# hpcaitech/CachedEmbedding

Hardware: AMD Instinct MI355X
Metric: embedding lookups/sec (cache op + EmbeddingBag fwd + bwd/SGD), Criteo-1TB table @1% cache (higher is better)
Workload: dtype f32

## Files before the change

cachedembedding_amd/_lib.py:

```python
from __future__ import annotations

import ctypes
import os
from ctypes import POINTER, Structure, c_char_p, c_double, c_float, c_int, c_int32, c_int64, c_size_t, c_uint64, c_void_p
from pathlib import Path

import torch

_PKG = Path(__file__).resolve().parent
LIB_PATH = Path(os.environ["CE_LIBRARY"]) if os.environ.get("CE_LIBRARY") else _PKG / "libce_hip.so"

CE_OK = 0
CE_ERR_INVALID = 1
CE_ERR_HIP = 2
CE_ERR_CAPACITY = 3
CE_ERR_NOMEM = 4
CE_ERR_UNSUPPORTED = 5
CE_ERR_RANGE = 6
CE_EVICT_DATASET = 0
CE_EVICT_LFU = 1
CE_EVICT_LRU = 2
CE_MODE_SUM = 0
CE_MODE_MEAN = 1
CE_ACT_F32 = 0
CE_ACT_BF16 = 1
CE_ACT_F16 = 2
CE_OPT_SGD = 0
CE_OPT_ROWWISE_ADAGRAD = 1
CE_ROUND_NEAREST = 0
CE_ROUND_STOCHASTIC = 1
CE_SORTED_CHUNK = 64
CE_COMPACT_BLOCK = 4096
CE_ACC_CACHE = 0
CE_ACC_STEP = 1
CE_WD_NONE = 0
CE_WD_L2 = 1
CE_WD_DECOUPLED = 2
CE_TRANSPORT_ZEROCOPY = 0
CE_TRANSPORT_STAGED = 1
CE_TRANSPORT_WORKER = 2
CE_CALL_PREPARE = 0
CE_CALL_PRELOAD = 1
CE_CALL_FLUSH = 2
CE_Q8_HEADER_BYTES = 16
CE_Q4_HEADER_BYTES = 16


class CeCacheConfig(Structure):
    _fields_ = [
        ("num_embeddings", c_int64),
        ("cuda_row_num", c_int64),
        ("embedding_dim", c_int32),
        ("evict_strategy", c_int32),
        ("transport", c_int32),
        ("protect_depth", c_int32),
        ("max_ids_per_call", c_int64),
        ("host_weight", c_void_p),
        ("host_weight_dev", c_void_p),
        ("cache_weight", c_void_p),
        ("idx_map", c_void_p),
        ("inverted_cached_idx", c_void_p),
        ("cached_idx_map", c_void_p),
        ("freq_cnter", c_void_p),
        ("workspace", c_void_p),
        ("workspace_bytes", c_size_t),
    ]


class CeCallStats(Structure):
    _fields_ = [
# ... 25 lines not shown
_WD = [c_float, c_int32]
_UPDATE_WD_TAIL = _KEYS + [c_void_p, c_void_p, c_int64, c_float, c_void_p, c_float] + _WD + \
    [c_int32, c_int32, c_uint64, c_int32, c_void_p, c_size_t] + _STREAM
_SORTED_WD_TAIL = [c_void_p, c_void_p, c_int64, c_float, c_float] + _WD + \
    [c_int32, c_int32, c_uint64, c_void_p, c_size_t] + _STREAM
_ADAM_WD_TAIL = _KEYS + [c_double, c_double, c_float, c_void_p, c_float] + _WD + \
    [c_void_p, c_int32, c_void_p, c_size_t] + _STREAM
_ROW_MOMENT = [c_void_p, c_void_p, c_int64]
_WINDOW = [c_void_p, c_int64, c_int64, c_int64]
_WINDOW_SRC = _WINDOW + [c_void_p, c_int32, c_int64, c_int64, c_int32, c_int64]
SIGNATURES = {
    "ce_version": (c_int, []),
    "ce_cpu_budget": (c_int32, []),
    "ce_last_error": (c_char_p, []),
    "ce_stream_create_cu_mask": (c_int, [c_void_p, c_int32, POINTER(c_void_p)]),
    "ce_stream_destroy": (c_int, [c_void_p]),
    "ce_host_alloc": (c_int, [c_size_t, c_int, POINTER(c_void_p), POINTER(c_void_p)]),
    "ce_host_free": (c_int, [c_void_p]),
    "ce_host_register": (c_int, [c_void_p, c_size_t, POINTER(c_void_p)]),
    "ce_host_unregister": (c_int, [c_void_p]),
    "ce_host_fill_uniform": (c_int, [c_void_p, c_int64, c_float, c_float, c_uint64, c_int]),
    "ce_host_fill_uniform_rows": (c_int, [c_void_p, c_int64, c_int32, c_float, c_float, c_uint64, c_void_p, c_void_p]),
    "ce_host_rows_gather": (c_int, [c_void_p, c_int64, c_int32, c_void_p, c_int64, c_void_p, c_void_p]),
    "ce_box_probe": (c_int, [c_void_p, c_size_t, c_int32, POINTER(c_double), POINTER(c_double), c_void_p]),
    "ce_probe_rows": (c_int, [c_void_p, c_int64, c_int32, c_int64, c_int32, POINTER(c_double), POINTER(c_double), c_void_p]),
    "ce_bag_forward": (c_int, _BAG + _STREAM),
    "ce_bag_backward_dense": (c_int, _BAG + _STREAM),
    "ce_bag_backward_dense_presorted": (c_int, _BAG + _KEYS + _STREAM),
    "ce_bag_backward_rows": (c_int, [c_void_p, c_void_p, c_int32, c_int64, c_void_p, c_int32, c_int64, c_int32, c_void_p,
                                     c_int32, c_int64, c_void_p, c_void_p]),
    "ce_bag_backward_sgd": (c_int, _BAG + [c_float] + _STREAM),
    "ce_bag_presort_len": (c_int64, [c_int64]),
    "ce_bag_presort": (c_int, [c_void_p, c_int64, c_int64, c_void_p, c_void_p]),
    "ce_bag_backward_sgd_presorted": (c_int, _BAG + [c_float] + _KEYS + _STREAM),
    "ce_bag_presort_window": (c_int, _WINDOW + _KEYS + _STREAM),
    "ce_bag_presort_window_src": (c_int, _WINDOW_SRC + _KEYS + _STREAM),
    "ce_bag_forward_src_keys": (c_int, _TABLE + [c_int64] + _KEYS + [c_void_p] + _STREAM),
    "ce_bag_backward_sgd_presorted_src": (c_int, _SRC + [c_float] + _KEYS + _STREAM),
    "ce_bag_presort_window_src_excl": (c_int, _WINDOW_SRC + [c_void_p] + _KEYS + [c_void_p] + _STREAM),
    "ce_bag_backward_sgd_presorted_src_excl": (c_int, _SRC + [c_float] + _KEYS + [c_void_p] + _STREAM),
    "ce_bag_backward_dense_presorted_src": (c_int, _SRC + _KEYS + _STREAM),
    "ce_bag_backward_sgd_sorted_workspace": (c_size_t, [c_int64, c_int64]),
    "ce_bag_backward_sgd_sorted": (c_int, _BAG + [c_float, c_void_p, c_size_t] + _STREAM),
    "ce_bag_backward_rowwise_adagrad_workspace": (c_size_t, [c_int64, c_int32]),
    "ce_bag_backward_rowwise_adagrad": (c_int, _BAG + _ADAGRAD_TAIL),
    "ce_bag_backward_rowwise_adagrad_src": (c_int, _SRC + _ADAGRAD_TAIL),
    "ce_bag_forward_act": (c_int, _BAG + _ACT + _STREAM),
    "ce_bag_forward_src_keys_act": (c_int, _TABLE + [c_int64] + _KEYS + [c_void_p] + _ACT + _STREAM),
    "ce_bag_backward_dense_act": (c_int, _BAG + _ACT + _KEYS + _STREAM),
    "ce_bag_backward_sgd_act": (c_int, _BAG + _ACT + [c_float] + _KEYS + _STREAM),
    "ce_bag_backward_sgd_src_act": (c_int, _SRC + _ACT + [c_float] + _KEYS + [c_void_p] + _STREAM),
    "ce_bag_backward_dense_src_act": (c_int, _SRC + _ACT + _KEYS + _STREAM),
    "ce_bag_backward_rowwise_adagrad_act": (c_int, _BAG + _ACT + _ADAGRAD_TAIL),
    "ce_bag_backward_rowwise_adagrad_src_act": (c_int, _SRC + _ACT + _ADAGRAD_TAIL),
    "ce_host_fill_uniform_w16": (c_int, [c_void_p, c_int64, c_float, c_float, c_uint64, c_int32, c_int]),
    "ce_bag_forward_w16": (c_int, _W16 + _BAG[1:] + _ACT + _STREAM),
    "ce_bag_forward_src_keys_w16": (c_int, _W16 + [c_int64, c_int32, c_int64] + _KEYS + [c_void_p] + _ACT + _STREAM),
    "ce_bag_backward_w16_workspace": (c_size_t, [c_int64, c_int32]),
    "ce_bag_backward_update_w16": (c_int, _W16 + _BAG[1:] + _ACT + _W16_TAIL),
    "ce_bag_backward_update_src_w16": (c_int, _W16 + _SRC[1:] + _ACT + _W16_TAIL),
    "ce_bag_backward_update_sorted_workspace": (c_size_t, [c_int64, c_int64, c_int32]),
    "ce_bag_backward_update_sorted": (c_int, _W16 + _BAG[1:] + _ACT + _W16_TAIL[1:]),
    "ce_bag_backward_update_compact_workspace": (c_size_t, [c_int64, c_int64, c_int32]),
    "ce_bag_backward_update_compact": (c_int, _W16 + _BAG[1:] + _ACT + _W16_TAIL),
    "ce_bag_backward_update_compact_src": (c_int, _W16 + _SRC[1:] + _ACT + _W16_TAIL),
    "ce_bag_backward_sgd_lrdev": (c_int, _BAG + _ACT + [c_void_p] + _KEYS + _STREAM),
# ... 256 lines not shown
```

cachedembedding_amd/csrc/ce_bag.hip:

```cpp
#include <algorithm>

#include "ce_common.h"

namespace ce {

struct BagParams {
  const float* weight;
  float* dst;
  const void* grad_out;
  const int64_t* indices;
  const void* offsets;
  const float* psw;
  int64_t nnz;
  int32_t num_bags;
  int32_t rowlen;
  int32_t g_log2;
  int32_t off64;
  int32_t include_last;
  int32_t mode;
  int32_t hookF;
  int32_t hookB;
  float alpha;
  int32_t pad0;
  uint32_t num_rows;
// ... 593 lines not shown
#pragma unroll
        for (int r = 0; r < kSegKeys; ++r) {
          const int e = r * 1024 + tid;
          if (e < n_here) {
            const long long v = ids[in_base + e];
            lo = v < lo ? v : lo;
            hi2 = v > hi2 ? v : hi2;
          }
        }
      } else {
        lo = INT64_MIN; hi2 = INT64_MAX;
      }
#pragma unroll
      for (int d = 32; d >= 1; d >>= 1) {
        const long long ol = __shfl_xor(lo, d), oh = __shfl_xor(hi2, d);
        lo = ol < lo ? ol : lo;
        hi2 = oh > hi2 ? oh : hi2;
      }
      if (lane == 0) { mm_s[0][wv] = lo; mm_s[1][wv] = hi2; }
      __syncthreads();
      if (tid == 0) {
        for (int k = 1; k < 16; ++k) {
          lo = mm_s[0][k] < lo ? mm_s[0][k] : lo;
          hi2 = mm_s[1][k] > hi2 ? mm_s[1][k] : hi2;
        }
        ids_minmax[2 * seg] = lo;
        ids_minmax[2 * seg + 1] = hi2;
      }
    }
    __syncthreads();
  }
}

template <typename VT, int NCH, typename KT, int R, typename AT, bool LRDEV = false>
__global__ __launch_bounds__(256) void k_bag_bwd_tile(BagParams p, const float* __restrict__ lr_dev) {
  using K = KeyOps<KT>;
  using A = Act<AT, VT>;
  __shared__ KT keys[kBwdTile];
  __shared__ int bagl[kBwdTile];
  __shared__ float scl[kBwdTile];

  const int tid = threadIdx.x;
  const int G = 1 << p.g_log2;
  const int ngroups = 256 >> p.g_log2;
  const int grp = tid >> p.g_log2;
  const int gl = tid & (G - 1);
  const int rowlen = p.rowlen;
  const int dim = rowlen * (int)(sizeof(VT) / 4);
  const typename A::V* __restrict__ GO = (const typename A::V*)p.grad_out;
  float alpha = p.alpha;
  if constexpr (LRDEV) alpha = -*lr_dev;
  const int tile_len = p.tile_len;
  const int64_t total = p.presorted ? ((p.nnz + kSegLen - 1) / kSegLen) * kSegLen : p.nnz;
  const int ntiles = (int)((total + tile_len - 1) / tile_len);

  for (int tile = blockIdx.x; tile < ntiles; tile += gridDim.x) {
    const int j0 = tile * tile_len;
    const int nv = min(tile_len, (int)(total - j0));
    const bool presorted = p.presorted != nullptr;
    KT kr[4];
#pragma unroll
    for (int r = 0; r < 4; ++r) {
      const int i = tid * 4 + r;
      kr[r] = K::invalid();
      int j = j0 + i;
      uint32_t row = 0xffffffffu;
      if (presorted) {
        const unsigned long long sk = i < nv ? p.presorted[(int64_t)j0 + i] : ~0ull;
        j = -1;
        if (sk != ~0ull) {
          row = (uint32_t)(sk >> 32);
          j = (int)((((int64_t)j0 + i) / kSegLen) * kSegLen) + (int)(uint32_t)sk;
        }
      } else if (i < nv) {
        const int64_t r64 = p.indices[j];
        if ((uint64_t)r64 < (uint64_t)p.num_rows) row = (uint32_t)r64;
      } else {
        j = -1;
      }
      const int bag = j >= 0 ? find_bag(p, j) : -1;
      if (bag >= 0) {
        float sc = alpha;
        if (p.psw) sc *= p.psw[j];
        if (p.mode == CE_MODE_MEAN) {
          const int len = bag_end(p, bag) - ld_off(p, bag);
          if (len > 1) sc = sc / (float)len;
        }
        bagl[i] = (int)out_row(p, bag);
        scl[i] = sc;
        if (row != 0xffffffffu) kr[r] = K::make(row, i);
      }
    }
    if (presorted) {
#pragma unroll
      for (int r = 0; r < 4; ++r) keys[tid * 4 + r] = kr[r];
      __syncthreads();
    } else {
      tile_sort_1024<KT>(kr, keys, tid);
    }
    const int kChunk = (nv + ngroups - 1) / ngroups;
    const int nchunks = (nv + kChunk - 1) / kChunk;
    for (int ck = grp; ck < nchunks; ck += ngroups) {
      const int s0 = ck * kChunk, s1 = min(nv, s0 + kChunk);
      VT acc[NCH];
#pragma unroll
      for (int c = 0; c < NCH; ++c) acc[c] = vzero<VT>();
      uint32_t cur = K::row(keys[s0]);
      for (int q = s0; q < s1; q += R) {
        VT v[R][NCH];
        float sc[R];
        uint32_t rw[R];
#pragma unroll
        for (int t = 0; t < R; ++t) {
          const KT key = (q + t < s1) ? keys[q + t] : K::invalid();
          const bool on = key != K::invalid();
          const int li = on ? K::idx(key) : 0;
          rw[t] = on ? K::row(key) : K::row_invalid();
          sc[t] = on ? scl[li] : 0.f;
          const int64_t orow = bagl[li];
#pragma unroll
          for (int c = 0; c < NCH; ++c) {
            const int ch = gl + c * G;
            v[t][c] = vzero<VT>();
            if (on && ch < rowlen) v[t][c] = A::up(__builtin_nontemporal_load(&GO[orow * rowlen + ch]));
          }
        }
        __builtin_amdgcn_s_waitcnt(0x0F70);
#pragma unroll
        for (int t = 0; t < R; ++t) {
          if (rw[t] != K::row_invalid()) {
            if (rw[t] != cur) {
#pragma unroll
              for (int c = 0; c < NCH; ++c) {
                if (cur != K::row_invalid())
                  flush_chunk(p.dst + (int64_t)cur * dim, acc[c], gl, G, c, rowlen);
                acc[c] = vzero<VT>();
              }
              cur = rw[t];
            }
#pragma unroll
            for (int c = 0; c < NCH; ++c) acc[c] = acc[c] + v[t][c] * sc[t];
          }
        }
      }
#pragma unroll
      for (int c = 0; c < NCH; ++c) {
        if (cur != K::row_invalid()) flush_chunk(p.dst + (int64_t)cur * dim, acc[c], gl, G, c, rowlen);
      }
    }
    __syncthreads();
  }
}

template <typename VT, int NCH, int R, bool EXCL, typename AT, bool PAIR = false, bool LRDEV = false>
__global__ __launch_bounds__(256) void k_bag_bwd_stream(BagParams p, int64_t total, const long long* __restrict__ seg_ranges,
                                                        const float* __restrict__ lr_dev) {
  using A = Act<AT, VT>;
  static_assert(!PAIR || (sizeof(typename A::V) == 8 && R % 2 == 0), "PAIR: 4 x 16 bit per lane, keys two at a time");
  __shared__ unsigned long long lk[256 * (R > 4 ? R : 4)];
  const int tid = threadIdx.x;
  const int G = 1 << p.g_log2;
  const int ngroups = 256 >> p.g_log2;
  const int grp = tid >> p.g_log2;
  const int gl = tid & (G - 1);
  const int rowlen = p.rowlen;
  const int dim = rowlen * (int)(sizeof(VT) / 4);
  const typename A::V* __restrict__ GO = (const typename A::V*)p.grad_out;
  const VT* __restrict__ WV = (const VT*)p.dst;
  const unsigned long long* __restrict__ keys = p.presorted;
  bool excl = false;
  if (EXCL) {
    const int nseg = (int)(total / kSegLen);
    int clash = nseg > 64 || seg_ranges == nullptr;
    if (!clash) {
      for (int pr = tid; pr < nseg * nseg; pr += 256) {
        const int a = pr / nseg, b2 = pr - a * nseg;
        if (a >= b2) continue;
        const long long alo = seg_ranges[2 * a], ahi = seg_ranges[2 * a + 1];
        const long long blo = seg_ranges[2 * b2], bhi = seg_ranges[2 * b2 + 1];
        if (alo <= ahi && blo <= bhi && !(ahi < blo || bhi < alo)) clash = 1;
      }
    }
    excl = __syncthreads_or(clash) == 0;
  }
  const int64_t all_groups = (int64_t)gridDim.x * ngroups;
  const int64_t round = R > 16 ? R : 16;
  const int64_t share = ((total + all_groups - 1) / all_groups + round - 1) / round * round;
  const int64_t s0 = share_of(p, grp, ngroups) * share;
  const int64_t s1 = min(total, s0 + share);
  if (s0 >= s1) return;
  float alpha = p.alpha;
  if constexpr (LRDEV) alpha = -*lr_dev;
// ... 76 lines not shown
                } else {
                  flush_chunk(p.dst + (int64_t)cur * dim, acc[c], gl, G, c, rowlen);
                }
              }
              acc[c] = EXCL ? w2[EXCL ? t : 0][c] : vzero<VT>();
            }
            cur = rw[t];
            cur_excl = head;
          }
#pragma unroll
          for (int c = 0; c < NCH; ++c) acc[c] = acc[c] + v[t][c] * alpha;
        }
      }
    }
  }
  if (cur != 0xffffffffu) {
#pragma unroll
    for (int c = 0; c < NCH; ++c) {
      if (EXCL && cur_excl) {
        const int ch = gl + c * G;
        if (ch < rowlen) ((VT*)(p.dst + (int64_t)cur * dim))[ch] = acc[c];
      } else {
        flush_chunk(p.dst + (int64_t)cur * dim, acc[c], gl, G, c, rowlen);
      }
    }
  }
}

template <typename VT, int NCH, int R, typename AT, bool PAIR = false, typename WT = float>
__global__ __launch_bounds__(256, 4) void k_bag_fwd_keys(BagParams p, int64_t total) {
  using A = Act<AT, VT>;
  using T = Row<WT, VT>;
  static_assert(!PAIR || (sizeof(typename A::V) == 8 && R % 2 == 0), "PAIR: 4 x 16 bit per lane, keys two at a time");
  __shared__ unsigned long long lk[256 * (R > 4 ? R : 4)];
  const int tid = threadIdx.x;
  const int G = 1 << p.g_log2;
  const int ngroups = 256 >> p.g_log2;
  const int grp = tid >> p.g_log2;
  const int gl = tid & (G - 1);
  const int rowlen = p.rowlen;
  const int stride = (T::kHeader + rowlen) * T::kSpan;
  const typename T::V* __restrict__ W = (const typename T::V*)p.weight;
  typename A::V* __restrict__ O = (typename A::V*)p.dst;
  const unsigned long long* __restrict__ keys = p.presorted;
  const int64_t all_groups = (int64_t)gridDim.x * ngroups;
  const int64_t round = R > 16 ? R : 16;
  const int64_t share = ((total + all_groups - 1) / all_groups + round - 1) / round * round;
  const int64_t s0 = share_of(p, grp, ngroups) * share;
  const int64_t s1 = min(total, s0 + share);
  if (s0 >= s1) return;
  const int kc = 4 * G > R ? 4 * G : R;
  unsigned long long* mylk = lk + grp * kc;
  VT prev[NCH];
#pragma unroll
  for (int c = 0; c < NCH; ++c) prev[c] = vzero<VT>();
  uint32_t prev_row = 0xffffffffu;
  for (int64_t c0 = s0; c0 < s1; c0 += kc) {
    for (int k = gl; k < kc; k += G) mylk[k] = c0 + k < s1 ? keys[c0 + k] : ~0ull;
    const int64_t c1 = min(s1, c0 + kc);
    for (int64_t q = c0; q < c1; q += R) {
      typename T::Held v[R][NCH];
      typename T::Hdr h[R];
      uint32_t heads = 0;
      uint32_t last = prev_row;
#pragma unroll
      for (int t = 0; t < R; ++t) {
        const unsigned long long k = mylk[(int)(q - c0) + t];
// ... 131 lines not shown
  p.g_log2 = r.g_log2;
  p.off64 = off64;
  p.include_last = include_last;
  p.mode = mode;
  p.hookF = (int32_t)hookF;
  p.hookB = hookF ? (int32_t)(num_bags / hookF) : 0;
  p.alpha = 1.f;
  p.num_rows = 0xffffffffu;
  return CE_OK;
}

static int fill_params_keys(BagParams& p, RowGeom& r, int32_t dim, bool aligned, int64_t nnz) {
  return fill_params(p, r, dim, aligned, nullptr, nnz, nullptr, 0, 0, 1, nullptr, CE_MODE_SUM, 0);
}

template <typename F> static void for_lanes_act(const RowGeom& r, int act, F&& f) {
  for_lanes(r.vec, r.nch, [&](auto l) { for_act(act, [&](auto a) { f(l, a); }); });
}
template <typename F> static void for_table_act(int weight_dtype, const RowGeom& r, int act, F&& f) {
  auto acts = [&](auto l, auto w) { for_act(act, [&](auto a) { f(l, w, a); }); };
  if (weight_dtype == kTableQ8) for_vec_lanes(r.nch, [&](auto l) { acts(l, ActTag<Q8>{}); });
  else if (weight_dtype == kTableQ4) for_vec_lanes(r.nch, [&](auto l) { acts(l, ActTag<Q4>{}); });
  else if (weight_dtype == kTableAdam) for_vec_lanes(r.nch, [&](auto l) { acts(l, ActTag<AdamRow>{}); });
  else if (weight_dtype == kTablePartialAdam)
    for_vec_lanes(r.nch, [&](auto l) { acts(l, ActTag<PartialAdamRow>{}); });
  else for_table(weight_dtype, r, acts);
}

template <typename VT, int NCH> constexpr int tile_unroll() {
  return NCH == 1 ? (sizeof(VT) == 16 ? 16 : 8) : (NCH == 2 ? 4 : 2);
}
template <typename VT, int NCH> constexpr int keys_unroll() { return NCH == 1 ? 16 : (NCH == 2 ? 8 : 4); }

template <typename VT, typename AT> constexpr bool kHasPair = sizeof(VT) == 16 && sizeof(AT) == 2;
static inline bool pair16(const RowGeom& r, int act, int32_t dim, const void* q) {
  return r.vec && act != CE_ACT_F32 && dim % 8 == 0 && al16(q);
}

static int bag_grid(int64_t num_bags) {
  int64_t tiles = cdiv(num_bags, 64);
  return grid_for(tiles, 4);
}

static int64_t padded_keys(int64_t nnz) { return cdiv(nnz, kSegLen) * kSegLen; }
static dim3 keys_grid(int64_t total, int g_log2, int per_cu) {
  const int ngroups = 256 >> g_log2;
  const int64_t shares = cdiv(total, (int64_t)ngroups * 16);
  return dim3((unsigned)std::max<int64_t>(1, std::min<int64_t>((int64_t)kNumCU * per_cu, shares)));
}

static int launch_bwd_scatter(BagParams& p, const RowGeom& r, int act, const float* lr_dev, hipStream_t s) {
  p.tile_len = kBwdTile;
  const int64_t total = p.presorted ? padded_keys(p.nnz) : p.nnz;
  if (p.presorted) {
    constexpr int per_cu = 2;
    if (total > (int64_t)kNumCU * 256)
      p.tile_len = (int)std::min<int64_t>(kBwdTile, (cdiv(total, (int64_t)kNumCU * per_cu) + 15) & ~15ll);
  }
  dim3 grid(std::min((int)cdiv(total, p.tile_len), kMaxBlocks)), block(256);
  const bool k32 = p.num_rows <= (1u << 22) - 2;
  for_lanes_act(r, act, [&](auto l, auto a) {
    using VT = typename decltype(l)::VT;
    using AT = typename decltype(a)::AT;
    constexpr int N = decltype(l)::NCH, R = tile_unroll<VT, N>();
    auto launch = [&](auto key, auto dev) {
      hipLaunchKernelGGL((k_bag_bwd_tile<VT, N, decltype(key), R, AT, decltype(dev)::value>), grid, block, 0, s, p, lr_dev);
// ... 14 lines not shown
  dim3 grid(bag_grid(p.num_bags)), block(256);
  const bool stage = p.nnz != p.num_bags;
  for_table_act(weight_dtype, r, act, [&](auto l, auto w, auto a) {
    using VT = typename decltype(l)::VT;
    using WT = typename decltype(w)::AT;
    using AT = typename decltype(a)::AT;
    constexpr int N = decltype(l)::NCH, U = tile_unroll<VT, N>();
    if (stage) hipLaunchKernelGGL((k_bag_fwd<VT, N, true, U, AT, WT>), grid, block, 0, s, p);
    else hipLaunchKernelGGL((k_bag_fwd<VT, N, false, U, AT, WT>), grid, block, 0, s, p);
  });
  CE_LAUNCH_CHECK();
  return CE_OK;
}

static int launch_fwd_keys(const void* weight, int weight_dtype, int64_t num_rows, int32_t dim, bool aligned, int64_t nnz,
                           const uint64_t* src_keys, void* out, int act, hipStream_t s) {
  BagParams p{};
  RowGeom r;
  int rc = fill_params_keys(p, r, dim, aligned, nnz);
  if (rc) return rc;
  p.weight = (const float*)weight;
  p.dst = (float*)out;
  p.num_rows = (uint32_t)num_rows;
  p.presorted = (const unsigned long long*)src_keys;
  p.interleave = 0;
  const int64_t total = padded_keys(nnz);
  const dim3 g = keys_grid(total, p.g_log2, 16), b(256);
  const bool pair = pair16(r, act, dim, out);
  for_table_act(weight_dtype, r, act, [&](auto l, auto w, auto a) {
    using VT = typename decltype(l)::VT;
    using WT = typename decltype(w)::AT;
    using AT = typename decltype(a)::AT;
    constexpr int N = decltype(l)::NCH, R = keys_unroll<VT, N>();
    if constexpr (std::is_same<WT, float>::value) {
      if constexpr (kHasPair<VT, AT>) {
        if (pair) {
          hipLaunchKernelGGL((k_bag_fwd_keys<VT, N, R, AT, true>), g, b, 0, s, p, total);
          return;
        }
      }
      hipLaunchKernelGGL((k_bag_fwd_keys<VT, N, R, AT>), g, b, 0, s, p, total);
    } else if constexpr (!std::is_same<AT, WT>::value) {
      hipLaunchKernelGGL((k_bag_fwd_keys<VT, N, R, AT, false, WT>), g, b, 0, s, p, total);
    }
  });
  CE_LAUNCH_CHECK();
  return CE_OK;
}

}

using namespace ce;

extern "C" int ce_bag_forward_act(const float* weight, int64_t num_rows, int32_t dim, const int64_t* indices,
                                  int64_t nnz, const void* offsets, int32_t offsets_are_i64, int64_t num_bags,
                                  int32_t include_last_offset, const float* per_sample_weights, int32_t mode,
                                  int64_t hook_features, void* out, int32_t act_dtype, ce_stream_t stream) {
  CE_REQUIRE_ACT(act_dtype);
  if (num_bags == 0) return CE_OK;
  CE_REQUIRE(weight && out && (indices || nnz == 0), CE_ERR_INVALID, "null pointer");
  CE_REQUIRE(offsets || num_bags == nnz, CE_ERR_INVALID,
             "offsets == NULL states one id per bag (offsets = arange): num_bags must equal nnz");
  BagParams p{};
  RowGeom r;
  int rc = fill_params(p, r, dim, al16(weight) && act_aligned(out, act_dtype), indices, nnz, offsets, offsets_are_i64,
                       num_bags, include_last_offset, per_sample_weights, mode, hook_features);
  if (rc) return rc;
  return launch_fwd(p, r, weight, CE_ACT_F32, num_rows, out, act_dtype, (hipStream_t)stream);
}

extern "C" int ce_bag_forward(const float* weight, int64_t num_rows, int32_t dim, const int64_t* indices,
                              int64_t nnz, const void* offsets, int32_t offsets_are_i64, int64_t num_bags,
                              int32_t include_last_offset, const float* per_sample_weights, int32_t mode,
                              int64_t hook_features, float* out, ce_stream_t stream) {
  return ce_bag_forward_act(weight, num_rows, dim, indices, nnz, offsets, offsets_are_i64, num_bags, include_last_offset,
                            per_sample_weights, mode, hook_features, out, CE_ACT_F32, stream);
// ... 94 lines not shown
  return backward_scatter_impl(weight, -lr, nullptr, num_rows, dim, indices, nnz, offsets, offsets_are_i64, num_bags,
                               include_last_offset, per_sample_weights, mode, hook_features, grad_out, CE_ACT_F32,
                               presorted_keys, stream);
}

static int launch_bwd_stream(float* dst, int64_t num_rows, int32_t dim, int64_t nnz, const void* grad_out, int act,
                             float alpha, const float* lr_dev, const uint64_t* keys, const int64_t* seg_ranges,
                             ce_stream_t stream) {
  CE_REQUIRE_ACT(act);
  if (nnz == 0) return CE_OK;
  CE_REQUIRE(dst && grad_out && keys, CE_ERR_INVALID, "null pointer");
  CE_REQUIRE_ROWS(num_rows);
  BagParams p{};
  RowGeom r;
  int rc = fill_params_keys(p, r, dim, al16(dst) && act_aligned(grad_out, act), nnz);
  if (rc) return rc;
  p.dst = dst;
  p.grad_out = grad_out;
  p.alpha = alpha;
  p.num_rows = (uint32_t)num_rows;
  p.presorted = (const unsigned long long*)keys;
  p.interleave = 1;
  const int64_t total = padded_keys(nnz);
  const dim3 g = keys_grid(total, p.g_log2, 6), b(256);
  hipStream_t s = (hipStream_t)stream;
  const long long* rg = (const long long*)seg_ranges;
  const bool excl = seg_ranges != nullptr;
  const bool pair = pair16(r, act, dim, grad_out);
  for_lanes_act(r, act, [&](auto l, auto a) {
    using VT = typename decltype(l)::VT;
    using AT = typename decltype(a)::AT;
    constexpr int N = decltype(l)::NCH, R = keys_unroll<VT, N>();
    constexpr bool has_excl = sizeof(VT) == 16 && N == 1, has_pair = kHasPair<VT, AT>;
    auto launch = [&](auto ex, auto pr) {
      constexpr bool EX = decltype(ex)::value, PR = decltype(pr)::value;
      if (lr_dev) hipLaunchKernelGGL((k_bag_bwd_stream<VT, N, R, EX, AT, PR, true>), g, b, 0, s, p, total, rg, lr_dev);
      else hipLaunchKernelGGL((k_bag_bwd_stream<VT, N, R, EX, AT, PR>), g, b, 0, s, p, total, rg, lr_dev);
    };
    if constexpr (has_excl && has_pair) { if (excl && pair) return launch(std::true_type{}, std::true_type{}); }
    if constexpr (has_excl) { if (excl) return launch(std::true_type{}, std::false_type{}); }
    if constexpr (has_pair) { if (pair) return launch(std::false_type{}, std::true_type{}); }
    launch(std::false_type{}, std::false_type{});
  });
  CE_LAUNCH_CHECK();
  return CE_OK;
}

extern "C" int ce_bag_backward_sgd_presorted_src(float* weight, int64_t num_rows, int32_t dim, int64_t nnz,
                                                 const float* grad_out, float lr, const uint64_t* src_keys,
                                                 ce_stream_t stream) {
  return launch_bwd_stream(weight, num_rows, dim, nnz, grad_out, CE_ACT_F32, -lr, nullptr, src_keys, nullptr, stream);
}

extern "C" int ce_bag_backward_sgd_presorted_src_excl(float* weight, int64_t num_rows, int32_t dim, int64_t nnz,
                                                      const float* grad_out, float lr, const uint64_t* src_keys,
                                                      const int64_t* seg_id_ranges, ce_stream_t stream) {
  return launch_bwd_stream(weight, num_rows, dim, nnz, grad_out, CE_ACT_F32, -lr, nullptr, src_keys, seg_id_ranges, stream);
}

extern "C" int ce_bag_backward_sgd_src_act(float* weight, int64_t num_rows, int32_t dim, int64_t nnz,
                                           const void* grad_out, int32_t act_dtype, float lr, const uint64_t* src_keys,
                                           const int64_t* seg_id_ranges, ce_stream_t stream) {
  return launch_bwd_stream(weight, num_rows, dim, nnz, grad_out, act_dtype, -lr, nullptr, src_keys, seg_id_ranges, stream);
}

extern "C" int ce_bag_backward_sgd_src_lrdev(float* weight, int64_t num_rows, int32_t dim, int64_t nnz,
                                             const void* grad_out, int32_t act_dtype, const float* lr,
                                             const uint64_t* src_keys, const int64_t* seg_id_ranges,
                                             ce_stream_t stream) {
  CE_REQUIRE(lr, CE_ERR_INVALID, "lr: null device pointer");
// ... 205 lines not shown
  CE_REQUIRE_ROWS(num_rows);
  CE_REQUIRE_ADAM_ALIGNED(weight, out, act_dtype);
  return launch_fwd_keys(weight, kTablePartialAdam, num_rows, dim, true, nnz, src_keys, out, act_dtype,
                         (hipStream_t)stream);
}

extern "C" int64_t ce_bag_presort_len(int64_t nnz) { return nnz <= 0 ? 0 : padded_keys(nnz); }

static int window_layout(BagParams& lay, const BagLayout& L, const int64_t* indices, int64_t nnz_per_batch) {
  CE_REQUIRE(L.num_bags > 0 && L.offsets_batch_stride >= 0, CE_ERR_INVALID, "bad offsets");
  CE_REQUIRE(L.offsets || L.num_bags == nnz_per_batch, CE_ERR_INVALID,
             "offsets may only be NULL for the one-id-per-bag layout (num_bags == nnz_per_batch)");
  RowGeom unused;
  return fill_params(lay, unused, 4, true, indices, nnz_per_batch, L.offsets, L.offsets_are_i64, L.num_bags,
                     L.include_last_offset, nullptr, CE_MODE_SUM, L.hook_features);
}

static int launch_presort(const int64_t* indices, int64_t* slots_io, const int32_t* inverted, const int* status,
                          int64_t nnz_per_batch, int64_t n_batches, int64_t num_rows, const BagLayout* L,
                          const int64_t* ids, int64_t* ids_minmax, uint64_t* keys_out, hipStream_t s) {
  if (nnz_per_batch == 0 || n_batches == 0) return CE_OK;
  CE_REQUIRE((slots_io ? inverted && status : indices != nullptr) && keys_out && nnz_per_batch > 0 && n_batches > 0,
             CE_ERR_INVALID, "bad arguments");
  CE_REQUIRE(nnz_per_batch < (int64_t)INT32_MAX - kSegLen, CE_ERR_INVALID, "batch too large");
  CE_REQUIRE_ROWS(num_rows);
  const int64_t spb = cdiv(nnz_per_batch, kSegLen);
  const int64_t nseg = spb * n_batches;
  CE_REQUIRE(spb < (int64_t)INT32_MAX && nseg < (int64_t)INT32_MAX, CE_ERR_INVALID, "too many segments");
  BagParams lay{};
  if (L) {
    int rc = window_layout(lay, *L, indices, nnz_per_batch);
    if (rc) return rc;
  }
  const dim3 grid((unsigned)std::min<int64_t>(nseg, kMaxBlocks)), block(1024);
  const int64_t off_stride = L ? L->offsets_batch_stride : 0;
  auto launch = [&](auto src, auto excl, auto rows) {
    hipLaunchKernelGGL((k_bag_presort_seg<decltype(src)::value, decltype(excl)::value, decltype(rows)::value>), grid, block,
                       0, s, indices, nnz_per_batch, (int32_t)spb, nseg, (uint32_t)num_rows,
                       (unsigned long long*)keys_out, lay, off_stride, ids, ids_minmax, slots_io, inverted, status);
  };
  const std::true_type yes{};
  const std::false_type no{};
  if (slots_io && L) launch(yes, no, yes);
  else if (slots_io) launch(no, no, yes);
  else if (L && ids_minmax) launch(yes, yes, no);
  else if (L) launch(yes, no, no);
  else launch(no, no, no);
  CE_LAUNCH_CHECK();
  return CE_OK;
}

namespace ce {
int presort_window_from_rows(int64_t* slots_io, int64_t nnz_per_batch, int64_t n_batches, int64_t num_rows,
                             const int32_t* inverted, const int* status, int32_t src_keys, const BagLayout& lay,
                             uint64_t* keys_out, hipStream_t stream) {
  return launch_presort(nullptr, slots_io, inverted, status, nnz_per_batch, n_batches, num_rows, src_keys ? &lay : nullptr,
                        nullptr, nullptr, keys_out, stream);
}
}

extern "C" int ce_bag_presort_window(const int64_t* indices, int64_t nnz_per_batch, int64_t n_batches,
                                     int64_t num_rows, uint64_t* keys_out, ce_stream_t stream) {
  return launch_presort(indices, nullptr, nullptr, nullptr, nnz_per_batch, n_batches, num_rows, nullptr, nullptr, nullptr,
                        keys_out, (hipStream_t)stream);
}

static int presort_window_src_impl(const int64_t* indices, int64_t nnz_per_batch, int64_t n_batches, int64_t num_rows,
                                   const BagLayout& L, const int64_t* ids, uint64_t* keys_out, int64_t* seg_id_ranges,
                                   ce_stream_t stream) {
  if (nnz_per_batch == 0 || n_batches == 0) return CE_OK;
  BagParams lay{};
  int rc = window_layout(lay, L, indices, nnz_per_batch);
  if (rc) return rc;
  return launch_presort(indices, nullptr, nullptr, nullptr, nnz_per_batch, n_batches, num_rows, &L, ids, seg_id_ranges,
                        keys_out, (hipStream_t)stream);
}

extern "C" int ce_bag_presort_window_src(const int64_t* indices, int64_t nnz_per_batch, int64_t n_batches,
                                         int64_t num_rows, const void* offsets, int32_t offsets_are_i64,
                                         int64_t offsets_batch_stride, int64_t num_bags, int32_t include_last_offset,
                                         int64_t hook_features, uint64_t* keys_out, ce_stream_t stream) {
  return presort_window_src_impl(indices, nnz_per_batch, n_batches, num_rows,
                                 {offsets, offsets_are_i64, offsets_batch_stride, num_bags, include_last_offset, hook_features},
                                 nullptr, keys_out, nullptr, stream);
}

extern "C" int ce_bag_presort_window_src_excl(const int64_t* indices, int64_t nnz_per_batch, int64_t n_batches,
                                              int64_t num_rows, const void* offsets, int32_t offsets_are_i64,
                                              int64_t offsets_batch_stride, int64_t num_bags,
                                              int32_t include_last_offset, int64_t hook_features, const int64_t* ids,
                                              uint64_t* keys_out, int64_t* seg_id_ranges, ce_stream_t stream) {
  CE_REQUIRE(seg_id_ranges, CE_ERR_INVALID, "null seg_id_ranges");
  return presort_window_src_impl(indices, nnz_per_batch, n_batches, num_rows,
                                 {offsets, offsets_are_i64, offsets_batch_stride, num_bags, include_last_offset, hook_features},
                                 ids, keys_out, seg_id_ranges, stream);
}

extern "C" int ce_bag_presort(const int64_t* indices, int64_t nnz, int64_t num_rows, uint64_t* keys_out,
                              ce_stream_t stream) {
  return ce_bag_presort_window(indices, nnz, 1, num_rows, keys_out, stream);
}

extern "C" int ce_rows_axpy(float* weight, int64_t num_rows, int32_t dim, const int64_t* index, int64_t n,
                            const float* src_rows, float alpha, ce_stream_t stream) {
  if (n == 0) return CE_OK;
  CE_REQUIRE(weight && index && src_rows, CE_ERR_INVALID, "null pointer");
  CE_REQUIRE(dim > 0 && n > 0 && n < (int64_t)INT32_MAX, CE_ERR_INVALID, "bad sizes");
  CE_REQUIRE_ROWS(num_rows);
  RowGeom r;
  int rc = row_geometry(dim, al16(weight) && al16(src_rows), r);
  if (rc) return rc;
  const int64_t per_block = (int64_t)(64 >> r.g_log2) * axpy_unroll(r.nch) * 4;
  dim3 grid(grid_for(n, (int)per_block)), block(256);
  hipStream_t s = (hipStream_t)stream;
  for_lanes(r.vec, r.nch, [&](auto l) {
    using VT = typename decltype(l)::VT;
    hipLaunchKernelGGL((k_rows_axpy<VT, decltype(l)::NCH>), grid, block, 0, s, weight, (uint32_t)num_rows, index, n,
                       (const VT*)src_rows, r.rowlen, r.g_log2, dim, alpha);
  });
  CE_LAUNCH_CHECK();
  return CE_OK;
}

extern "C" int ce_bag_backward_rows(float* grad_rows, const int64_t* dest_index, int32_t dim, int64_t nnz,
                                    const void* offsets, int32_t offsets_are_i64, int64_t num_bags,
                                    int32_t include_last_offset, const float* per_sample_weights, int32_t mode,
                                    int64_t hook_features, const float* grad_out, ce_stream_t stream) {
  if (num_bags == 0 || nnz == 0) return CE_OK;
  CE_REQUIRE(grad_rows && grad_out && offsets, CE_ERR_INVALID, "null pointer");
  BagParams p{};
  RowGeom r;
  int rc = fill_params(p, r, dim, al16(grad_rows) && al16(grad_out), dest_index, nnz, offsets, offsets_are_i64,
                       num_bags, include_last_offset, per_sample_weights, mode, hook_features);
// ... 13 lines not shown
```

include/ce_api.h:

```cpp
#ifndef CE_API_H
#define CE_API_H

#include <stddef.h>
#include <stdint.h>

#ifdef __cplusplus
extern "C" {
#endif

#define CE_API_VERSION 6

#define CE_OK 0
#define CE_ERR_INVALID 1
#define CE_ERR_HIP 2
#define CE_ERR_CAPACITY 3
#define CE_ERR_NOMEM 4
#define CE_ERR_UNSUPPORTED 5
#define CE_ERR_RANGE 6

#define CE_EVICT_DATASET 0
#define CE_EVICT_LFU 1
#define CE_EVICT_LRU 2

#define CE_MODE_SUM 0
// ... 27 lines not shown
int ce_host_rows_gather(const float* table_dev, int64_t num_rows, int32_t dim, const int64_t* rows, int64_t n,
                        float* out, ce_stream_t stream);
int ce_box_probe(void* scratch, size_t bytes, int32_t reps, double* read_GBps, double* fill_GBps, ce_stream_t stream);
int ce_probe_rows(float* buf, int64_t rows, int32_t dim, int64_t fold, int32_t reps, double* write_us, double* read_us,
                  ce_stream_t stream);

int ce_bag_forward(const float* weight, int64_t num_rows, int32_t dim,
                   const int64_t* indices, int64_t nnz,
                   const void* offsets, int32_t offsets_are_i64, int64_t num_bags,
                   int32_t include_last_offset, const float* per_sample_weights, int32_t mode,
                   int64_t hook_features, float* out, ce_stream_t stream);

int ce_bag_backward_dense(float* grad_weight, int64_t num_rows, int32_t dim,
                          const int64_t* indices, int64_t nnz,
                          const void* offsets, int32_t offsets_are_i64, int64_t num_bags,
                          int32_t include_last_offset, const float* per_sample_weights, int32_t mode,
                          int64_t hook_features, const float* grad_out, ce_stream_t stream);

int ce_bag_backward_rows(float* grad_rows, const int64_t* dest_index, int32_t dim, int64_t nnz,
                         const void* offsets, int32_t offsets_are_i64, int64_t num_bags,
                         int32_t include_last_offset, const float* per_sample_weights, int32_t mode,
                         int64_t hook_features, const float* grad_out, ce_stream_t stream);

int ce_bag_backward_sgd(float* weight, int64_t num_rows, int32_t dim,
                        const int64_t* indices, int64_t nnz,
                        const void* offsets, int32_t offsets_are_i64, int64_t num_bags,
                        int32_t include_last_offset, const float* per_sample_weights, int32_t mode,
                        int64_t hook_features, const float* grad_out, float lr, ce_stream_t stream);

int64_t ce_bag_presort_len(int64_t nnz);
int ce_bag_presort(const int64_t* indices, int64_t nnz, int64_t num_rows, uint64_t* keys_out, ce_stream_t stream);
int ce_bag_presort_window(const int64_t* indices, int64_t nnz_per_batch, int64_t n_batches, int64_t num_rows,
                          uint64_t* keys_out, ce_stream_t stream);
int ce_bag_backward_sgd_presorted(float* weight, int64_t num_rows, int32_t dim,
                                  const int64_t* indices, int64_t nnz,
                                  const void* offsets, int32_t offsets_are_i64, int64_t num_bags,
                                  int32_t include_last_offset, const float* per_sample_weights, int32_t mode,
                                  int64_t hook_features, const float* grad_out, float lr,
                                  const uint64_t* presorted_keys, ce_stream_t stream);
int ce_bag_backward_dense_presorted(float* grad_weight, int64_t num_rows, int32_t dim,
                                    const int64_t* indices, int64_t nnz,
                                    const void* offsets, int32_t offsets_are_i64, int64_t num_bags,
                                    int32_t include_last_offset, const float* per_sample_weights, int32_t mode,
                                    int64_t hook_features, const float* grad_out,
                                    const uint64_t* presorted_keys, ce_stream_t stream);
int ce_bag_presort_window_src(const int64_t* indices, int64_t nnz_per_batch, int64_t n_batches, int64_t num_rows,
                              const void* offsets, int32_t offsets_are_i64, int64_t offsets_batch_stride,
                              int64_t num_bags, int32_t include_last_offset, int64_t hook_features,
                              uint64_t* keys_out, ce_stream_t stream);
int ce_bag_forward_src_keys(const float* weight, int64_t num_rows, int32_t dim, int64_t nnz, const uint64_t* src_keys,
                            float* out, ce_stream_t stream);
int ce_bag_backward_sgd_presorted_src(float* weight, int64_t num_rows, int32_t dim, int64_t nnz,
                                      const float* grad_out, float lr, const uint64_t* src_keys, ce_stream_t stream);
int ce_bag_backward_dense_presorted_src(float* grad_weight, int64_t num_rows, int32_t dim, int64_t nnz,
                                        const float* grad_out, const uint64_t* src_keys, ce_stream_t stream);
int ce_bag_presort_window_src_excl(const int64_t* indices, int64_t nnz_per_batch, int64_t n_batches, int64_t num_rows,
                                   const void* offsets, int32_t offsets_are_i64, int64_t offsets_batch_stride,
                                   int64_t num_bags, int32_t include_last_offset, int64_t hook_features,
                                   const int64_t* ids, uint64_t* keys_out, int64_t* seg_id_ranges,
                                   ce_stream_t stream);
int ce_bag_backward_sgd_presorted_src_excl(float* weight, int64_t num_rows, int32_t dim, int64_t nnz,
                                           const float* grad_out, float lr, const uint64_t* src_keys,
                                           const int64_t* seg_id_ranges, ce_stream_t stream);

size_t ce_bag_backward_sgd_sorted_workspace(int64_t num_rows, int64_t nnz);
int ce_bag_backward_sgd_sorted(float* weight, int64_t num_rows, int32_t dim,
// ... 384 lines not shown
```

Baseline: 3.216 billion.

## Add slim 512-thread presort kernel and size keys-kernel LDS dynamically

Replaces the 1024-thread segment presort with a 512-thread counting-sort variant. It keeps per-key bucket and place packed in registers, uses wave-aggregated atomics when a whole wave hits one bucket, and writes keys out in two halves through half-size LDS, with the counters aliased into the key buffer. The forward and backward keys kernels switch from fixed static shared arrays to dynamic shared memory sized from the group geometry, so their LDS footprint and occupancy can shrink. A footprint query entry point is added to report registers and LDS. The gain is higher occupancy and less LDS pressure, at the cost of re-reading indices in the output pass and a more intricate sort path.

```diff
diff --git a/cachedembedding_amd/_lib.py b/cachedembedding_amd/_lib.py
--- a/cachedembedding_amd/_lib.py
+++ b/cachedembedding_amd/_lib.py
@@ -36,6 +36,9 @@
 CE_WD_NONE = 0
 CE_WD_L2 = 1
 CE_WD_DECOUPLED = 2
+CE_KERNEL_PRESORT = 0
+CE_KERNEL_FWD_KEYS = 1
+CE_KERNEL_BWD_STREAM = 2
 CE_TRANSPORT_ZEROCOPY = 0
 CE_TRANSPORT_STAGED = 1
 CE_TRANSPORT_WORKER = 2
@@ -127,6 +130,7 @@
     "ce_bag_backward_sgd": (c_int, _BAG + [c_float] + _STREAM),
     "ce_bag_presort_len": (c_int64, [c_int64]),
     "ce_bag_presort": (c_int, [c_void_p, c_int64, c_int64, c_void_p, c_void_p]),
+    "ce_bag_kernel_footprint": (c_int, [c_int32, POINTER(c_int32), POINTER(c_int32), POINTER(c_int32)]),
     "ce_bag_backward_sgd_presorted": (c_int, _BAG + [c_float] + _KEYS + _STREAM),
     "ce_bag_presort_window": (c_int, _WINDOW + _KEYS + _STREAM),
     "ce_bag_presort_window_src": (c_int, _WINDOW_SRC + _KEYS + _STREAM),
diff --git a/cachedembedding_amd/csrc/ce_bag.hip b/cachedembedding_amd/csrc/ce_bag.hip
--- a/cachedembedding_amd/csrc/ce_bag.hip
+++ b/cachedembedding_amd/csrc/ce_bag.hip
@@ -649,6 +649,171 @@
   }
 }
 
+constexpr int kSlimThreads = 512;
+constexpr int kSlimKeys = kSegLen / kSlimThreads;
+constexpr int kSlimChunk = 8;
+constexpr int kSlimOut = 4;
+constexpr int kSlimHalf = kSegLen / 2;
+constexpr int kSlimBktBits = 14;
+static_assert(kSegBuckets < (1 << kSlimBktBits) && kSegLen <= (1 << (32 - kSlimBktBits)), "bucket | place in 32 bits");
+static_assert(kSegBuckets % kSlimThreads == 0 && (kSegBuckets + 1 + kSlimThreads / 64) * sizeof(int) <= kSlimHalf * sizeof(unsigned long long),
+              "the counters alias the key buffer");
+
+constexpr int kSrcNone = 0, kSrcStated = 1, kSrcOffsets = 2;
+
+__device__ __forceinline__ uint32_t slot32(int64_t slot, uint32_t num_rows) {
+  return (uint64_t)slot < (uint64_t)num_rows ? (uint32_t)slot : 0xffffffffu;
+}
+template <int SRC>
+__device__ __forceinline__ unsigned long long presort_key(const BagParams& q, int sib, int e, int n_here, uint32_t s) {
+  if (e >= n_here) return ~0ull;
+  if (!SRC) return s != 0xffffffffu ? ((unsigned long long)s << 32) | (unsigned)e : ~0ull;
+  int bag = sib * kSegLen + e;
+  if (SRC == kSrcOffsets) {
+    bag = find_bag(q, bag);
+    if (bag < 0) return ~0ull;
+  }
+  return ((unsigned long long)s << 32) | (unsigned)out_row(q, bag);
+}
+
+template <int SRC, bool ROWS>
+__global__ __launch_bounds__(kSlimThreads) __attribute__((amdgpu_waves_per_eu(5)))
+void k_bag_presort_seg_slim(const int64_t* __restrict__ indices, int64_t nnz_per_batch, int32_t segs_per_batch,
+                            int64_t n_segs, uint32_t num_rows, unsigned long long* __restrict__ keys_out, BagParams lay,
+                            int64_t off_stride, int64_t* slots_io, const int32_t* __restrict__ inverted,
+                            const int* __restrict__ status) {
+  extern __shared__ unsigned long long lk[];
+  int* const cnt = (int*)lk;
+  int* const wsum = cnt + kSegBuckets + 1;
+  const int tid = threadIdx.x, lane = tid & 63, wv = tid >> 6;
+  for (int64_t seg = blockIdx.x; seg < n_segs; seg += gridDim.x) {
+    const int64_t batch = seg / segs_per_batch;
+    const int sib = (int)(seg - batch * segs_per_batch);
+    const int64_t in_base = batch * nnz_per_batch + (int64_t)sib * kSegLen;
+    const int64_t base = seg * kSegLen;
+    const int n_here = (int)min((int64_t)kSegLen, nnz_per_batch - (int64_t)sib * kSegLen);
+    BagParams q = lay;
+    if (SRC == kSrcOffsets) q.offsets = (const char*)lay.offsets + batch * off_stride * (lay.off64 ? 8 : 4);
+    for (int i = tid; i <= kSegBuckets; i += kSlimThreads) cnt[i] = 0;
+    __syncthreads();
+    uint32_t w[kSlimKeys];
+    const bool failed = ROWS && *status != CE_OK;
+#pragma unroll
+    for (int c = 0; c < kSlimKeys; c += kSlimChunk) {
+      int t = tid;
+      asm volatile("" : "+v"(t));
+      uint32_t s[kSlimChunk];
+      if (ROWS) {
+        int32_t row[kSlimChunk];
+#pragma unroll
+        for (int u = 0; u < kSlimChunk; ++u) {
+          const int e = (c + u) * kSlimThreads + t;
+          row[u] = (int32_t)slots_io[in_base + (e < n_here ? e : 0)];
+        }
+#pragma unroll
+        for (int u = 0; u < kSlimChunk; ++u) {
+          const int e = (c + u) * kSlimThreads + t;
+          const bool look = e < n_here && row[u] >= 0 && !failed;
+          row[u] = inverted[look ? row[u] : 0];
+          if (!look) row[u] = -1;
+        }
+#pragma unroll
+        for (int u = 0; u < kSlimChunk; ++u) {
+          const int e = (c + u) * kSlimThreads + t;
+          if (e < n_here) slots_io[in_base + e] = (int64_t)row[u];
+          s[u] = slot32((int64_t)row[u], num_rows);
+        }
+      } else {
+#pragma unroll
+        for (int u = 0; u < kSlimChunk; ++u) {
+          const int e = (c + u) * kSlimThreads + t;
+          s[u] = slot32(indices[in_base + (e < n_here ? e : 0)], num_rows);
+          if (e >= n_here) s[u] = 0xffffffffu;
+        }
+      }
+      int place[kSlimChunk];
+#pragma unroll
+      for (int u = 0; u < kSlimChunk; ++u) {
+        int bkt = kSegBuckets;
+        if (s[u] != 0xffffffffu) {
+          bool covered = true;
+          if (SRC == kSrcOffsets) covered = find_bag(q, sib * kSegLen + (c + u) * kSlimThreads + t) >= 0;
+          if (covered) bkt = (int)(s[u] & (kSegBuckets - 1));
+        }
+        s[u] = (uint32_t)bkt;
+        const int b0 = __builtin_amdgcn_readfirstlane(bkt);
+        if (__all(bkt == b0)) {
+          int first = 0;
+          if (lane == 0) first = atomicAdd(&cnt[b0], 64);
+          place[u] = __builtin_amdgcn_readfirstlane(first) + lane;
+        } else {
+          place[u] = atomicAdd(&cnt[bkt], 1);
+        }
+      }
+#pragma unroll
+      for (int u = 0; u < kSlimChunk; ++u) {
+        w[c + u] = s[u] | ((uint32_t)place[u] << kSlimBktBits);
+        asm volatile("" : "+v"(w[c + u]));
+      }
+    }
+    __syncthreads();
+    constexpr int kPer = kSegBuckets / kSlimThreads;
+    int sum = 0;
+#pragma unroll
+    for (int k = 0; k < kPer; ++k) sum += cnt[tid * kPer + k];
+    int inc = sum;
+#pragma unroll
+    for (int d = 1; d < 64; d <<= 1) {
+      const int o = __shfl_up(inc, d);
+      if (lane >= d) inc += o;
+    }
+    if (lane == 63) wsum[wv] = inc;
+    __syncthreads();
+    int pre = inc - sum;
+    for (int k = 0; k < wv; ++k) pre += wsum[k];
+    int total = 0;
+    for (int k = 0; k < kSlimThreads / 64; ++k) total += wsum[k];
+#pragma unroll
+    for (int k = 0; k < kPer; ++k) {
+      const int n = cnt[tid * kPer + k];
+      cnt[tid * kPer + k] = pre;
+      pre += n;
+    }
+    if (tid == 0) cnt[kSegBuckets] = total;
+    __syncthreads();
+#pragma unroll
+    for (int r = 0; r < kSlimKeys; ++r) w[r] = (uint32_t)cnt[w[r] & ((1u << kSlimBktBits) - 1)] + (w[r] >> kSlimBktBits);
+    __syncthreads();
+#pragma unroll 1
+    for (int h = 0; h < kSegLen / kSlimHalf; ++h) {
+      int t = tid;
+      asm volatile("" : "+v"(t));
+#pragma unroll
+      for (int c = 0; c < kSlimKeys; c += kSlimOut) {
+        uint32_t s[kSlimOut];
+#pragma unroll
+        for (int u = 0; u < kSlimOut; ++u) {
+          const int e = (c + u) * kSlimThreads + t;
+          const int64_t at = in_base + (e < n_here ? e : 0);
+          typedef int32_t __attribute__((may_alias)) low_word;
+          s[u] = ROWS ? slot32((int64_t)((const low_word*)slots_io)[2 * at], num_rows) : slot32(indices[at], num_rows);
+        }
+#pragma unroll
+        for (int u = 0; u < kSlimOut; ++u) {
+          const int e = (c + u) * kSlimThreads + t;
+          const int pos = (int)w[c + u];
+          if (pos / kSlimHalf == h) lk[pos % kSlimHalf] = presort_key<SRC>(q, sib, e, n_here, s[u]);
+        }
+      }
+      __syncthreads();
+#pragma unroll
+      for (int k = 0; k < kSlimHalf / kSlimThreads; ++k)
+        keys_out[base + h * kSlimHalf + k * kSlimThreads + t] = lk[k * kSlimThreads + t];
+      __syncthreads();
+    }
+  }
+}
+
 template <typename VT, int NCH, typename KT, int R, typename AT, bool LRDEV = false>
 __global__ __launch_bounds__(256) void k_bag_bwd_tile(BagParams p, const float* __restrict__ lr_dev) {
   using K = KeyOps<KT>;
@@ -715,10 +880,10 @@
     } else {
       tile_sort_1024<KT>(kr, keys, tid);
     }
-    const int kChunk = (nv + ngroups - 1) / ngroups;
-    const int nchunks = (nv + kChunk - 1) / kChunk;
+    const int kSlimChunk = (nv + ngroups - 1) / ngroups;
+    const int nchunks = (nv + kSlimChunk - 1) / kSlimChunk;
     for (int ck = grp; ck < nchunks; ck += ngroups) {
-      const int s0 = ck * kChunk, s1 = min(nv, s0 + kChunk);
+      const int s0 = ck * kSlimChunk, s1 = min(nv, s0 + kSlimChunk);
       VT acc[NCH];
 #pragma unroll
       for (int c = 0; c < NCH; ++c) acc[c] = vzero<VT>();
@@ -774,7 +939,7 @@
                                                         const float* __restrict__ lr_dev) {
   using A = Act<AT, VT>;
   static_assert(!PAIR || (sizeof(typename A::V) == 8 && R % 2 == 0), "PAIR: 4 x 16 bit per lane, keys two at a time");
-  __shared__ unsigned long long lk[256 * (R > 4 ? R : 4)];
+  extern __shared__ unsigned long long lk[];
   const int tid = threadIdx.x;
   const int G = 1 << p.g_log2;
   const int ngroups = 256 >> p.g_log2;
@@ -917,7 +1082,7 @@
   using A = Act<AT, VT>;
   using T = Row<WT, VT>;
   static_assert(!PAIR || (sizeof(typename A::V) == 8 && R % 2 == 0), "PAIR: 4 x 16 bit per lane, keys two at a time");
-  __shared__ unsigned long long lk[256 * (R > 4 ? R : 4)];
+  extern __shared__ unsigned long long lk[];
   const int tid = threadIdx.x;
   const int G = 1 << p.g_log2;
   const int ngroups = 256 >> p.g_log2;
@@ -1115,6 +1280,11 @@
 }
 template <typename VT, int NCH> constexpr int keys_unroll() { return NCH == 1 ? 16 : (NCH == 2 ? 8 : 4); }
 
+static size_t keys_lds_bytes(int g_log2, int R) {
+  const int G = 1 << g_log2;
+  return (size_t)(256 >> g_log2) * std::max(4 * G, R) * sizeof(unsigned long long);
+}
+
 template <typename VT, typename AT> constexpr bool kHasPair = sizeof(VT) == 16 && sizeof(AT) == 2;
 static inline bool pair16(const RowGeom& r, int act, int32_t dim, const void* q) {
   return r.vec && act != CE_ACT_F32 && dim % 8 == 0 && al16(q);
@@ -1195,16 +1365,17 @@
     using WT = typename decltype(w)::AT;
     using AT = typename decltype(a)::AT;
     constexpr int N = decltype(l)::NCH, R = keys_unroll<VT, N>();
+    const size_t lds = keys_lds_bytes(p.g_log2, R);
     if constexpr (std::is_same<WT, float>::value) {
       if constexpr (kHasPair<VT, AT>) {
         if (pair) {
-          hipLaunchKernelGGL((k_bag_fwd_keys<VT, N, R, AT, true>), g, b, 0, s, p, total);
+          hipLaunchKernelGGL((k_bag_fwd_keys<VT, N, R, AT, true>), g, b, lds, s, p, total);
           return;
         }
       }
-      hipLaunchKernelGGL((k_bag_fwd_keys<VT, N, R, AT>), g, b, 0, s, p, total);
+      hipLaunchKernelGGL((k_bag_fwd_keys<VT, N, R, AT>), g, b, lds, s, p, total);
     } else if constexpr (!std::is_same<AT, WT>::value) {
-      hipLaunchKernelGGL((k_bag_fwd_keys<VT, N, R, AT, false, WT>), g, b, 0, s, p, total);
+      hipLaunchKernelGGL((k_bag_fwd_keys<VT, N, R, AT, false, WT>), g, b, lds, s, p, total);
     }
   });
   CE_LAUNCH_CHECK();
@@ -1365,10 +1536,11 @@
     using AT = typename decltype(a)::AT;
     constexpr int N = decltype(l)::NCH, R = keys_unroll<VT, N>();
     constexpr bool has_excl = sizeof(VT) == 16 && N == 1, has_pair = kHasPair<VT, AT>;
+    const size_t lds = keys_lds_bytes(p.g_log2, R);
     auto launch = [&](auto ex, auto pr) {
       constexpr bool EX = decltype(ex)::value, PR = decltype(pr)::value;
-      if (lr_dev) hipLaunchKernelGGL((k_bag_bwd_stream<VT, N, R, EX, AT, PR, true>), g, b, 0, s, p, total, rg, lr_dev);
-      else hipLaunchKernelGGL((k_bag_bwd_stream<VT, N, R, EX, AT, PR>), g, b, 0, s, p, total, rg, lr_dev);
+      if (lr_dev) hipLaunchKernelGGL((k_bag_bwd_stream<VT, N, R, EX, AT, PR, true>), g, b, lds, s, p, total, rg, lr_dev);
+      else hipLaunchKernelGGL((k_bag_bwd_stream<VT, N, R, EX, AT, PR>), g, b, lds, s, p, total, rg, lr_dev);
     };
     if constexpr (has_excl && has_pair) { if (excl && pair) return launch(std::true_type{}, std::true_type{}); }
     if constexpr (has_excl) { if (excl) return launch(std::true_type{}, std::false_type{}); }
@@ -1640,20 +1812,24 @@
     int rc = window_layout(lay, *L, indices, nnz_per_batch);
     if (rc) return rc;
   }
-  const dim3 grid((unsigned)std::min<int64_t>(nseg, kMaxBlocks)), block(1024);
+  const dim3 grid((unsigned)std::min<int64_t>(nseg, kMaxBlocks));
   const int64_t off_stride = L ? L->offsets_batch_stride : 0;
-  auto launch = [&](auto src, auto excl, auto rows) {
-    hipLaunchKernelGGL((k_bag_presort_seg<decltype(src)::value, decltype(excl)::value, decltype(rows)::value>), grid, block,
-                       0, s, indices, nnz_per_batch, (int32_t)spb, nseg, (uint32_t)num_rows,
-                       (unsigned long long*)keys_out, lay, off_stride, ids, ids_minmax, slots_io, inverted, status);
+  auto launch = [&](auto src, auto rows) {
+    hipLaunchKernelGGL((k_bag_presort_seg_slim<decltype(src)::value, decltype(rows)::value>), grid, dim3(kSlimThreads),
+                       kSlimHalf * sizeof(unsigned long long), s, indices, nnz_per_batch, (int32_t)spb, nseg,
+                       (uint32_t)num_rows, (unsigned long long*)keys_out, lay, off_stride, slots_io, inverted, status);
   };
-  const std::true_type yes{};
-  const std::false_type no{};
-  if (slots_io && L) launch(yes, no, yes);
-  else if (slots_io) launch(no, no, yes);
-  else if (L && ids_minmax) launch(yes, yes, no);
-  else if (L) launch(yes, no, no);
-  else launch(no, no, no);
+  auto launch_src = [&](auto rows) {
+    if (!L) launch(std::integral_constant<int, kSrcNone>{}, rows);
+    else if (!lay.offsets) launch(std::integral_constant<int, kSrcStated>{}, rows);
+    else launch(std::integral_constant<int, kSrcOffsets>{}, rows);
+  };
+  if (slots_io) launch_src(std::true_type{});
+  else if (L && ids_minmax)
+    hipLaunchKernelGGL((k_bag_presort_seg<true, true, false>), grid, dim3(1024), 0, s, indices, nnz_per_batch, (int32_t)spb,
+                       nseg, (uint32_t)num_rows, (unsigned long long*)keys_out, lay, off_stride, ids, ids_minmax, slots_io,
+                       inverted, status);
+  else launch_src(std::false_type{});
   CE_LAUNCH_CHECK();
   return CE_OK;
 }
@@ -1707,6 +1883,32 @@
 extern "C" int ce_bag_presort(const int64_t* indices, int64_t nnz, int64_t num_rows, uint64_t* keys_out,
                               ce_stream_t stream) {
   return ce_bag_presort_window(indices, nnz, 1, num_rows, keys_out, stream);
+}
+
+extern "C" int ce_bag_kernel_footprint(int32_t kernel, int32_t* num_regs, int32_t* shared_bytes, int32_t* max_threads) {
+  CE_REQUIRE(num_regs && shared_bytes && max_threads, CE_ERR_INVALID, "null pointer");
+  constexpr int kDim = 128, R = keys_unroll<f32x4, 1>();
+  BagParams p{};
+  RowGeom r;
+  int rc = fill_params_keys(p, r, kDim, true, kSegLen);
+  if (rc) return rc;
+  const void* fn = nullptr;
+  size_t dynamic = keys_lds_bytes(p.g_log2, R);
+  switch (kernel) {
+    case CE_KERNEL_PRESORT:
+      fn = (const void*)k_bag_presort_seg_slim<kSrcStated, true>;
+      dynamic = kSlimHalf * sizeof(unsigned long long);
+      break;
+    case CE_KERNEL_FWD_KEYS: fn = (const void*)k_bag_fwd_keys<f32x4, 1, R, float>; break;
+    case CE_KERNEL_BWD_STREAM: fn = (const void*)k_bag_bwd_stream<f32x4, 1, R, false, float>; break;
+    default: CE_REQUIRE(false, CE_ERR_INVALID, "unknown kernel %d", (int)kernel);
+  }
+  hipFuncAttributes a{};
+  CE_HIP_CHECK(hipFuncGetAttributes(&a, fn));
+  *num_regs = a.numRegs;
+  *shared_bytes = (int32_t)(a.sharedSizeBytes + dynamic);
+  *max_threads = a.maxThreadsPerBlock;
+  return CE_OK;
 }
 
 extern "C" int ce_rows_axpy(float* weight, int64_t num_rows, int32_t dim, const int64_t* index, int64_t n,
diff --git a/include/ce_api.h b/include/ce_api.h
--- a/include/ce_api.h
+++ b/include/ce_api.h
@@ -83,6 +83,10 @@
 int ce_bag_presort(const int64_t* indices, int64_t nnz, int64_t num_rows, uint64_t* keys_out, ce_stream_t stream);
 int ce_bag_presort_window(const int64_t* indices, int64_t nnz_per_batch, int64_t n_batches, int64_t num_rows,
                           uint64_t* keys_out, ce_stream_t stream);
+#define CE_KERNEL_PRESORT 0
+#define CE_KERNEL_FWD_KEYS 1
+#define CE_KERNEL_BWD_STREAM 2
+int ce_bag_kernel_footprint(int32_t kernel, int32_t* num_regs, int32_t* shared_bytes, int32_t* max_threads);
 int ce_bag_backward_sgd_presorted(float* weight, int64_t num_rows, int32_t dim,
                                   const int64_t* indices, int64_t nnz,
                                   const void* offsets, int32_t offsets_are_i64, int64_t num_bags,
```

Result: no change. 3.222 billion, median of 5 (+0.2%).
